# dluvizon/deephar

Hardware: AMD Instinct MI355X
Metric: frames/sec whole-node, 256x256 MPII pose fwd (higher is better)
Workload: dtype f32; 1 GPU; MPII single-person 256x256, ReceptionNet 8 blocks J=16 ctx=2 k=5, pose-only forward, batch=64 per GPU (BASELINE.json configs[1]); global_batch=64, parallelism=frame-shard x1 (replicas, no collective), hipgraph=True, streams=1, input=f32, gemm=f32, outputs_finite_in_range=True

## Files before the change

### deephar_amd/csrc/conv_common.h

```cpp
#pragma once
#include <type_traits>

#include "dh_kernels.h"

namespace dh {

typedef float f32x16 __attribute__((ext_vector_type(16)));
typedef float f32x4v __attribute__((ext_vector_type(4)));

__device__ __forceinline__ void st4_stream(float* ptr, float4 v) {
  f32x4v t = {v.x, v.y, v.z, v.w};
  __builtin_nontemporal_store(t, reinterpret_cast<f32x4v*>(ptr));
}
__device__ __forceinline__ float4 ld4_stream(const float* ptr) {
  const f32x4v t = __builtin_nontemporal_load(reinterpret_cast<const f32x4v*>(ptr));
  return make_float4(t.x, t.y, t.z, t.w);
}

template <typename RSRC>
__device__ __forceinline__ float buf_ld1_stream(RSRC rs, int voff, int soff) {
  float r = 0.f;
#if defined(__HIP_DEVICE_COMPILE__)
  r = __uint_as_float(__builtin_amdgcn_raw_buffer_load_b32(rs, voff, soff, 2));
#endif
  return r;
}
template <typename RSRC>
__device__ __forceinline__ void buf_st1_stream(RSRC rs, int voff, int soff, float v) {
#if defined(__HIP_DEVICE_COMPILE__)
  __builtin_amdgcn_raw_buffer_store_b32(__float_as_uint(v), rs, voff, soff, 2);
#endif
}
__device__ __forceinline__ float& f4c(float4& v, int c) { return c == 0 ? v.x : c == 1 ? v.y : c == 2 ? v.z : v.w; }
__device__ __forceinline__ float f4c(const float4& v, int c) { return c == 0 ? v.x : c == 1 ? v.y : c == 2 ? v.z : v.w; }

__device__ __forceinline__ int xcd_tile(int b, int nwg) {
  const int xcd = b & 7, q = nwg >> 3, r = nwg & 7;
  return (xcd < r ? xcd * (q + 1) : r * (q + 1) + (xcd - r) * q) + (b >> 3);
}

template <int TM, int TN>
struct EpiPrefetch {
  static constexpr int ROW4 = TN * 8;
  static constexpr int IT = 4 * TN;
  static constexpr bool kEnabled = (TM == 1);
  float4 r1[kEnabled ? TM : 1][kEnabled ? IT : 1];
  float dsc[kEnabled ? TN : 1], dsh[kEnabled ? TN : 1];

  template <int WM, int WN>
  static __device__ __forceinline__ bool direct_tile(const ConvArgs& p, int m0, int n0, int M, int epi_vec) {
    return (epi_vec & 2) != 0 && m0 + WM * TM * 32 <= M && n0 + WN * TN * 32 <= p.Cout;
  }

  template <int WM, int WN>
  __device__ __forceinline__ void issue(const ConvArgs& p, int m0, int n0, int M, int epi_vec) {
    if constexpr (kEnabled) {
      if (direct_tile<WM, WN>(p, m0, n0, M, epi_vec)) {
        const int lane = threadIdx.x & 63, wave = threadIdx.x >> 6;
        const int wm = wave / WN, wn = wave % WN;
        const int li = lane & 31, lh = lane >> 5;
        const int ncol = n0 + wn * TN * 32 + li;
        if (p.post_scale != nullptr) {
#pragma unroll
          for (int j = 0; j < TN; ++j) { dsc[j] = p.post_scale[ncol + j * 32]; dsh[j] = p.post_shift[ncol + j * 32]; }
        }
        if (p.res1 == nullptr) return;
        const auto rs = __builtin_amdgcn_make_buffer_rsrc(const_cast<float*>(p.res1), 0,
                                                          (int)(((unsigned)(M - 1) * p.ldr1 + (unsigned)p.Cout) * 4u), 0x00020000);
        const int vo = ((m0 + wm * TM * 32 + 4 * lh) * p.ldr1 + ncol) * 4;
#pragma unroll
        for (int i = 0; i < TM; ++i)
#pragma unroll
          for (int j = 0; j < TN; ++j)
#pragma unroll
            for (int r = 0; r < 16; ++r)
              f4c(r1[i][j * 4 + (r >> 2)], r & 3) = buf_ld1_stream(rs, vo, ((i * 32 + (r & 3) + 8 * (r >> 2)) * p.ldr1 + j * 32) * 4);
        return;
      }
      if (epi_vec == 0 || p.res1 == nullptr) return;
      const int lane = threadIdx.x & 63, wave = threadIdx.x >> 6;
      const int wm = wave / WN, wn = wave % WN;
#pragma unroll
      for (int i = 0; i < TM; ++i)
#pragma unroll
        for (int it = 0; it < IT; ++it) {
          const int f = lane + 64 * it;
          const int row = f / ROW4, c4 = f - row * ROW4;
          int m = m0 + (wm * TM + i) * 32 + row;
          int n = n0 + wn * TN * 32 + c4 * 4;
          m = m < M ? m : M - 1;
          n = n < p.Cout ? n : p.Cout - 4;
          r1[i][it] = ld4_stream(p.res1 + (size_t)m * p.ldr1 + n);
        }
    }
  }
};

struct EpiNoHook {
  __device__ __forceinline__ void operator()() const {}
};

template <int WM, int WN, int TM, int TN, bool UP2, bool PRE, typename HOOK = EpiNoHook, bool DIRECT_R2 = true, int CHROWS = 0>
__device__ __forceinline__ void conv_epilogue(const ConvArgs& p, f32x16 (&acc)[TM][TN], float* smem, int m0,
                                              int n0, int M, int epi_vec, const EpiPrefetch<TM, TN>& pre,
                                              HOOK staged = HOOK()) {
  const int tid = threadIdx.x;
  const int lane = tid & 63;
  const int wave = tid >> 6;
  const int wm = wave / WN, wn = wave % WN;
  const int li = lane & 31, lh = lane >> 5;
  constexpr int LDC = TN * 32 + 4;
  constexpr int ROW4 = TN * 8;
  constexpr int IT = 4 * TN;
  constexpr int NSC = (64 % ROW4 == 0) ? 1 : 3;
  constexpr bool kPre = PRE && EpiPrefetch<TM, TN>::kEnabled;
  constexpr bool kPool = tile_pools_in_pairs(WM, TM, UP2);
  constexpr bool kPoolWave = tile_pools_in_wave(TM, UP2);
  if constexpr (!UP2 && kPre && std::is_same<HOOK, EpiNoHook>::value) {
    if (EpiPrefetch<TM, TN>::template direct_tile<WM, WN>(p, m0, n0, M, epi_vec)) {
      const auto rs_y = __builtin_amdgcn_make_buffer_rsrc(p.y, 0, (int)(((unsigned)(M - 1) * p.ldy + (unsigned)p.Cout) * 4u),
                                                          0x00020000);
      const int ncol = n0 + wn * TN * 32 + li;
      const int vo = ((m0 + wm * TM * 32 + 4 * lh) * p.ldy + ncol) * 4;
      float sc[TN], sh[TN];
#pragma unroll
      for (int j = 0; j < TN; ++j) {
        sc[j] = pre.dsc[j];
        sh[j] = pre.dsh[j];
      }
      float r2[DIRECT_R2 ? TN : 1][8];
      if (DIRECT_R2 && p.res2 != nullptr) {
        const auto rs_2 = __builtin_amdgcn_make_buffer_rsrc(
            const_cast<float*>(p.res2), 0, (int)(((unsigned)((M >> 2) - 1) * p.ldr2 + (unsigned)p.Cout) * 4u), 0x00020000);
        const int ohw = p.OH * p.OW, ow_sh = __ffs(p.OW) - 1;
        const int mb = __builtin_amdgcn_readfirstlane(m0 + wm * 32);
        const int fr = mb >> (__ffs(ohw) - 1), pos = mb & (ohw - 1);
        const int oh0 = pos >> ow_sh, ow0 = pos & (p.OW - 1);
        const int v2 = (2 * lh * p.ldr2 + ncol) * 4;
#pragma unroll
        for (int j = 0; j < TN; ++j)
#pragma unroll
          for (int h = 0; h < 8; ++h) {
            const int tr = 2 * (h & 1) + 8 * (h >> 1);
            const int oh = oh0 + (tr >> ow_sh), ow = ow0 + (tr & (p.OW - 1));
            const int src = (fr * (p.OH >> 1) + (oh >> 1)) * (p.OW >> 1) + (ow >> 1);
            r2[j][h] = buf_ld1_stream(rs_2, v2, (src * p.ldr2 + j * 32) * 4);
          }
      }
#pragma unroll
      for (int i = 0; i < TM; ++i)
#pragma unroll
        for (int j = 0; j < TN; ++j)
#pragma unroll
          for (int r = 0; r < 16; ++r) {
            float t = acc[i][j][r];
            if (p.post_scale != nullptr) t = t * sc[j] + sh[j];
            if (p.res1 != nullptr) t += f4c(pre.r1[i][j * 4 + (r >> 2)], r & 3);
            if (DIRECT_R2 && p.res2 != nullptr) t += r2[DIRECT_R2 ? j : 0][r >> 1];
            if (p.post_relu) t = fmaxf(t, 0.f);
            buf_st1_stream(rs_y, vo, ((i * 32 + (r & 3) + 8 * (r >> 2)) * p.ldy + j * 32) * 4, t);
          }
      return;
    }
  }
  float* sC = smem + wave * 32 * LDC;
  const int ohw = p.OH * p.OW;
  const bool vec = epi_vec != 0;
  const bool pow2 = (p.OW & (p.OW - 1)) == 0 && (ohw & (ohw - 1)) == 0;
  const int ow_sh = __ffs(p.OW) - 1, ohw_sh = __ffs(ohw) - 1;
  __syncthreads();
#pragma unroll
  for (int i = 0; i < TM; ++i) {
    if (i > 0) asm volatile("s_waitcnt lgkmcnt(0)" ::: "memory");
#pragma unroll
    for (int j = 0; j < TN; ++j)
#pragma unroll
      for (int r = 0; r < 16; ++r)
        sC[((r & 3) + 8 * (r >> 2) + 4 * lh) * LDC + j * 32 + li] = acc[i][j][r];
    asm volatile("s_waitcnt lgkmcnt(0)" ::: "memory");
    if (i == TM - 1) staged();
    if (vec) {
      float4 rr[kPre ? 1 : IT], sc[NSC], sh[NSC];
      int ncol[NSC];
#pragma unroll
      for (int q = 0; q < NSC; ++q) {
        const int c4 = (lane + 64 * q) % ROW4;
        const int n = n0 + wn * TN * 32 + c4 * 4;
        ncol[q] = n < p.Cout ? n : p.Cout - 4;
        if (p.post_scale != nullptr) {
          sc[q] = *reinterpret_cast<const float4*>(p.post_scale + ncol[q]);
          sh[q] = *reinterpret_cast<const float4*>(p.post_shift + ncol[q]);
        }
      }
      if constexpr (!kPre && CHROWS == 0) {
        if (p.res1 != nullptr) {
#pragma unroll
          for (int it = 0; it < IT; ++it) {
            const int row = (lane + 64 * it) / ROW4;
            const int m = m0 + (wm * TM + i) * 32 + row;
            rr[it] = ld4_stream(p.res1 + (size_t)(m < M ? m : M - 1) * p.ldr1 + ncol[it % NSC]);
          }
        }
      }
      constexpr int CH = UP2 ? (IT < 4 ? IT : 4) : (CHROWS > 0 && CHROWS < IT ? CHROWS : IT);
      static_assert(IT % CH == 0, "chunks of equal size");
      constexpr int ND = UP2 ? 4 : 1;
#pragma unroll
      for (int c0 = 0; c0 < IT; c0 += CH) {
        float4 r2[CH][ND];
        size_t mo[CH][ND];
        if constexpr (!kPre && CHROWS > 0) {
          if (p.res1 != nullptr) {
#pragma unroll
            for (int u = 0; u < CH; ++u) {
              const int row = (lane + 64 * (c0 + u)) / ROW4;
              const int m = m0 + (wm * TM + i) * 32 + row;
              rr[c0 + u] = ld4_stream(p.res1 + (size_t)(m < M ? m : M - 1) * p.ldr1 + ncol[(c0 + u) % NSC]);
            }
          }
        }
#pragma unroll
        for (int u = 0; u < CH; ++u) {
          const int it = c0 + u;
          const int row = (lane + 64 * it) / ROW4;
          const int m = m0 + (wm * TM + i) * 32 + row;
          const int mc = m < M ? m : M - 1;
          if constexpr (UP2) {
            int fr, oh, ow;
            if (pow2) {
              fr = mc >> ohw_sh;
              const int rem = mc & (ohw - 1);
              oh = rem >> ow_sh;
              ow = rem & (p.OW - 1);
            } else {
              fr = mc / ohw;
              const int rem = mc - fr * ohw;
              oh = rem / p.OW;
              ow = rem - oh * p.OW;
            }
#pragma unroll
            for (int d = 0; d < 4; ++d)
              mo[u][d] = ((size_t)fr * 2 * p.OH + 2 * oh + (d >> 1)) * (2 * p.OW) + 2 * ow + (d & 1);
          } else {
            mo[u][0] = (size_t)mc;
          }
          if (p.res2 != nullptr) {
            if (!UP2 && p.res2_down) {
              int fr, oh, ow;
              if (pow2) {
                fr = mc >> ohw_sh;
                const int rem = mc & (ohw - 1);
                oh = rem >> ow_sh;
                ow = rem & (p.OW - 1);
              } else {
                fr = mc / ohw;
                const int rem = mc - fr * ohw;
                oh = rem / p.OW;
                ow = rem - oh * p.OW;
              }
              const size_t mr = ((size_t)fr * (p.OH >> 1) + (oh >> 1)) * (p.OW >> 1) + (ow >> 1);
              r2[u][0] = *reinterpret_cast<const float4*>(p.res2 + mr * p.ldr2 + ncol[it % NSC]);
            } else {
#pragma unroll
              for (int d = 0; d < ND; ++d)
                r2[u][d] = ld4_stream(p.res2 + mo[u][d] * p.ldr2 + ncol[it % NSC]);
            }
          }
        }
#pragma unroll
        for (int u = 0; u < CH; ++u) {
          const int it = c0 + u;
          const int f = lane + 64 * it;
          const int row = f / ROW4, c4 = f - row * ROW4;
          const int m = m0 + (wm * TM + i) * 32 + row;
          const int nc = ncol[it % NSC];
          const bool ok = m < M && n0 + wn * TN * 32 + c4 * 4 < p.Cout;
          float4 t = *reinterpret_cast<const float4*>(&sC[row * LDC + c4 * 4]);
          if (p.post_scale != nullptr) {
            const float4 a = sc[it % NSC], b = sh[it % NSC];
            t.x = t.x * a.x + b.x; t.y = t.y * a.y + b.y; t.z = t.z * a.z + b.z; t.w = t.w * a.w + b.w;
          }
          if (p.res1 != nullptr) {
            float4 r;
            if constexpr (kPre) r = pre.r1[i][it]; else r = rr[it];
            t.x += r.x; t.y += r.y; t.z += r.z; t.w += r.w;
          }
#pragma unroll
          for (int d = 0; d < ND; ++d) {
            float4 o = t;
            if (p.res2 != nullptr) { o.x += r2[u][d].x; o.y += r2[u][d].y; o.z += r2[u][d].z; o.w += r2[u][d].w; }
            if (p.post_relu) {
              o.x = fmaxf(o.x, 0.f); o.y = fmaxf(o.y, 0.f); o.z = fmaxf(o.z, 0.f); o.w = fmaxf(o.w, 0.f);
            }
            if (ok) st4_stream(p.y + mo[u][d] * p.ldy + nc, o);
            if constexpr (kPool || kPoolWave) {
              if (p.y_pool != nullptr) *reinterpret_cast<float4*>(&sC[row * LDC + c4 * 4]) = o;
            }
          }
        }
      }
    } else {
      for (int f = lane; f < 32 * ROW4; f += 64) {
        const int row = f / ROW4, c4 = f - row * ROW4;
        const int m = m0 + (wm * TM + i) * 32 + row;
        const int n = n0 + wn * TN * 32 + c4 * 4;
        if (m >= M || n >= p.Cout) continue;
        const float4 v = *reinterpret_cast<const float4*>(&sC[row * LDC + c4 * 4]);
        size_t mo[4];
        int nout = 1;
        if constexpr (UP2) {
          const int fr = m / ohw;
          const int rem = m - fr * ohw;
          const int oh = rem / p.OW, ow = rem - oh * p.OW;
#pragma unroll
          for (int d = 0; d < 4; ++d)
            mo[d] = ((size_t)fr * 2 * p.OH + 2 * oh + (d >> 1)) * (2 * p.OW) + 2 * ow + (d & 1);
          nout = 4;
        } else {
          mo[0] = (size_t)m;
        }
#pragma unroll
        for (int e = 0; e < 4; ++e) {
          if (n + e >= p.Cout) break;
          float t = (&v.x)[e];
          if (p.post_scale != nullptr) t = t * p.post_scale[n + e] + p.post_shift[n + e];
          if (p.res1 != nullptr) t += p.res1[(size_t)m * p.ldr1 + n + e];
          for (int d = 0; d < nout; ++d) {
            float o = t;
            if (p.res2 != nullptr) {
              size_t mr = mo[d];
              if (!UP2 && p.res2_down) {
                const int fr = m / ohw;
                const int rem = m - fr * ohw;
                const int oh = rem / p.OW, ow = rem - oh * p.OW;
                mr = ((size_t)fr * (p.OH >> 1) + (oh >> 1)) * (p.OW >> 1) + (ow >> 1);
              }
              o += p.res2[mr * p.ldr2 + n + e];
            }
            if (p.post_relu) o = fmaxf(o, 0.f);
            p.y[mo[d] * p.ldy + n + e] = o;
          }
        }
      }
    }
  }
  if constexpr (kPool) {
    if (p.y_pool != nullptr && vec && p.OW == 32) {
      __syncthreads();
      const float* sE = smem + ((wm & ~1) * WN + wn) * 32 * LDC;
      const float* sO = sE + WN * 32 * LDC;
      const int r_img = m0 / 32 + (wm & ~1);
      if ((r_img + 2) * 32 <= M) {
        const int fr = r_img / p.OH, oh = r_img - fr * p.OH;
        const size_t pp = ((size_t)fr * (p.OH / 2) + oh / 2) * 16;
        for (int idx = (wm & 1) * 64 + lane; idx < 16 * ROW4; idx += 128) {
          const int q = idx / ROW4, c4 = idx - q * ROW4;
          const int n = n0 + wn * TN * 32 + c4 * 4;
          if (n >= p.Cout) continue;
          const float4 a = *reinterpret_cast<const float4*>(&sE[(2 * q) * LDC + c4 * 4]);
          const float4 b = *reinterpret_cast<const float4*>(&sE[(2 * q + 1) * LDC + c4 * 4]);
          const float4 c = *reinterpret_cast<const float4*>(&sO[(2 * q) * LDC + c4 * 4]);
          const float4 d = *reinterpret_cast<const float4*>(&sO[(2 * q + 1) * LDC + c4 * 4]);
          float4 t;
          t.x = fmaxf(fmaxf(a.x, b.x), fmaxf(c.x, d.x)); t.y = fmaxf(fmaxf(a.y, b.y), fmaxf(c.y, d.y));
          t.z = fmaxf(fmaxf(a.z, b.z), fmaxf(c.z, d.z)); t.w = fmaxf(fmaxf(a.w, b.w), fmaxf(c.w, d.w));
          *reinterpret_cast<float4*>(p.y_pool + (pp + q) * p.ldyp + n) = t;
        }
      }
      __syncthreads();
    }
  }
  if constexpr (kPoolWave) {
    if (p.y_pool != nullptr && vec && p.OW < 32) {
      asm volatile("s_waitcnt lgkmcnt(0)" ::: "memory");
      const int mb = m0 + wm * 32;
      if (mb + 32 <= M) {
        const int pw_sh = __ffs(p.OW) - 2;
        const int row0 = mb >> (pw_sh + 1);
        const int fr = row0 / p.OH, oh = row0 - fr * p.OH;
        const size_t pp = ((size_t)fr * (p.OH >> 1) + (oh >> 1)) << pw_sh;
        for (int idx = lane; idx < 8 * ROW4; idx += 64) {
          const int q = idx / ROW4, c4 = idx - q * ROW4;
          const int n = n0 + wn * TN * 32 + c4 * 4;
          if (n >= p.Cout) continue;
          const int pr = q >> pw_sh, pc = q & ((1 << pw_sh) - 1);
          const float* s0 = sC + ((2 * pr) * p.OW + 2 * pc) * LDC + c4 * 4;
          const float4 a = *reinterpret_cast<const float4*>(s0);
          const float4 b = *reinterpret_cast<const float4*>(s0 + LDC);
          const float4 c = *reinterpret_cast<const float4*>(s0 + p.OW * LDC);
          const float4 d = *reinterpret_cast<const float4*>(s0 + (p.OW + 1) * LDC);
          float4 t;
          t.x = fmaxf(fmaxf(a.x, b.x), fmaxf(c.x, d.x)); t.y = fmaxf(fmaxf(a.y, b.y), fmaxf(c.y, d.y));
          t.z = fmaxf(fmaxf(a.z, b.z), fmaxf(c.z, d.z)); t.w = fmaxf(fmaxf(a.w, b.w), fmaxf(c.w, d.w));
          *reinterpret_cast<float4*>(p.y_pool + (pp + q) * p.ldyp + n) = t;
        }
      }
      asm volatile("s_waitcnt lgkmcnt(0)" ::: "memory");
    }
  }
}

template <int WM, int WN, int TM, int TN>
__device__ __forceinline__ void d2s_epilogue(const ConvArgs& p, f32x16 (&acc)[TM][TN], float* smem, const int m0, const int n0,
                                             const int M, const int vec, const int cb) {
  const int lane = threadIdx.x & 63, wave = threadIdx.x >> 6;
  const int wm = wave / WN, wn = wave % WN;
  const int li = lane & 31, lh = lane >> 5;
  constexpr int LDC = TN * 32 + 4, ROW4 = TN * 8, IT = 4 * TN;
  float* sC = smem + wave * 32 * LDC;
  const int hw = p.OH * p.OW;
  const bool pow2 = (p.OW & (p.OW - 1)) == 0 && (hw & (hw - 1)) == 0;
  const int ow_sh = __ffs(p.OW) - 1, hw_sh = __ffs(hw) - 1;
  auto out_pixel = [&](int m, int q) {
    int fr, oh, ow;
    if (pow2) {
      fr = m >> hw_sh;
      const int rem = m & (hw - 1);
      oh = rem >> ow_sh;
      ow = rem & (p.OW - 1);
    } else {
      fr = m / hw;
      const int rem = m - fr * hw;
      oh = rem / p.OW;
      ow = rem - oh * p.OW;
    }
    return ((size_t)fr * 2 * p.OH + 2 * oh + (q >> 1)) * (2 * p.OW) + 2 * ow + (q & 1);
  };
  __syncthreads();
#pragma unroll
  for (int i = 0; i < TM; ++i) {
    if (i > 0) asm volatile("s_waitcnt lgkmcnt(0)" ::: "memory");
#pragma unroll
    for (int j = 0; j < TN; ++j)
#pragma unroll
      for (int r = 0; r < 16; ++r) sC[((r & 3) + 8 * (r >> 2) + 4 * lh) * LDC + j * 32 + li] = acc[i][j][r];
    asm volatile("s_waitcnt lgkmcnt(0)" ::: "memory");
    if (vec) {
      constexpr int CH = IT < 4 ? IT : 4;
#pragma unroll
      for (int c0 = 0; c0 < IT; c0 += CH) {
        float4 rr[CH];
        size_t mo[CH];
        int co[CH];
        bool ok[CH];
#pragma unroll
        for (int u = 0; u < CH; ++u) {
          const int f = lane + 64 * (c0 + u);
          const int row = f / ROW4, c4 = f - row * ROW4;
          const int m = m0 + (wm * TM + i) * 32 + row;
          const int n = n0 + wn * TN * 32 + c4 * 4;
          ok[u] = m < M && n < p.Cout;
          const int mc = ok[u] ? m : 0, nc = ok[u] ? n : 0;
          const int q = (nc >= cb) + (nc >= 2 * cb) + (nc >= 3 * cb);
          co[u] = nc - q * cb;
          mo[u] = out_pixel(mc, q);
          if (p.res1 != nullptr) rr[u] = ld4_stream(p.res1 + mo[u] * p.ldr1 + co[u]);
        }
#pragma unroll
        for (int u = 0; u < CH; ++u) {
          const int f = lane + 64 * (c0 + u);
          const int row = f / ROW4, c4 = f - row * ROW4;
          float4 t = *reinterpret_cast<const float4*>(&sC[row * LDC + c4 * 4]);
          if (p.res1 != nullptr) { t.x += rr[u].x; t.y += rr[u].y; t.z += rr[u].z; t.w += rr[u].w; }
          if (p.post_relu) { t.x = fmaxf(t.x, 0.f); t.y = fmaxf(t.y, 0.f); t.z = fmaxf(t.z, 0.f); t.w = fmaxf(t.w, 0.f); }
          if (ok[u]) st4_stream(p.y + mo[u] * p.ldy + co[u], t);
        }
      }
    } else {
      for (int f = lane; f < 32 * TN * 32; f += 64) {
        const int row = f / (TN * 32), c = f - row * (TN * 32);
        const int m = m0 + (wm * TM + i) * 32 + row;
        const int n = n0 + wn * TN * 32 + c;
        if (m >= M || n >= p.Cout) continue;
        const int q = (n >= cb) + (n >= 2 * cb) + (n >= 3 * cb);
        const int ch = n - q * cb;
        const size_t mo = out_pixel(m, q);
        float t = sC[row * LDC + c];
        if (p.res1 != nullptr) t += p.res1[mo * p.ldr1 + ch];
        if (p.post_relu) t = fmaxf(t, 0.f);
        p.y[mo * p.ldy + ch] = t;
      }
    }
  }
}

}
```

### deephar_amd/csrc/gemm1x1_body.h

```cpp
#pragma once
#include "conv_common.h"
#include "gemm_family.h"
#include "lds_dma.h"

namespace dh {

template <bool PRE, int S>
__device__ __forceinline__ void fetch_affine(unsigned t_sc, unsigned t_sh, float4& sc, float4& sh) {
  if constexpr (PRE) {
    sc = lds_rd<S * 32>(t_sc);
    sh = lds_rd<S * 32>(t_sh);
  }
}

template <int TM, int TN, int BN, int BOFF, int S>
__device__ __forceinline__ void fetch_frags(const unsigned (&a_addr)[TM][4], unsigned b_addr, float4 (&fa)[TM],
                                            float4 (&fb)[TN]) {
  fa[0] = lds_rd<0>(a_addr[0][S]);
  if constexpr (TM > 1) fa[1] = lds_rd<0>(a_addr[1][S]);
  constexpr int BO = BOFF + S * 2 * BN * 16;
  fb[0] = lds_rd<BO>(b_addr);
  if constexpr (TN > 1) fb[1] = lds_rd<BO + 512>(b_addr);
  if constexpr (TN > 2) fb[2] = lds_rd<BO + 1024>(b_addr);
}

template <int WM, int WN, int TM, int TN, bool UP2, bool RELU, bool KXK = false, bool PRE = false, bool D2S = false>
__device__ __forceinline__ void gemm1x1_body(const ConvArgs& p, const int epi_vec, const int block, const int nblocks,
                                             float* const smem, const int cb = 0) {
  static_assert(!(PRE && (KXK || UP2)), "the BN prologue is built for the plain pointwise form");
  static_assert(!(D2S && (KXK || UP2)), "the depth-to-space epilogue follows the plain pointwise main loop");
  constexpr int NT = WM * WN * 64;
  constexpr int BM = WM * TM * 32;
  constexpr int BN = WN * TN * 32;
  constexpr int APASS = BM * 8 / NT;
  constexpr int BPASS = 8 * BN / NT;
  constexpr int STAGE = BM * BK + BK * BN;
  static_assert(BM * 8 % NT == 0 && (8 * BN) % NT == 0, "tile/thread mismatch");

  const int tid = threadIdx.x;
  const int lane = tid & 63;
  const int wave = tid >> 6;
  const int wm = wave / WN, wn = wave % WN;
  const int li = lane & 31, lh = lane >> 5;

  const int M = p.N * p.OH * p.OW;
  const int tiles_n = (p.Cout + BN - 1) / BN;
  const int tile = xcd_tile(block, nblocks);
  const int m0 = (tile / tiles_n) * BM;
  const int n0 = (tile % tiles_n) * BN;

  const int wave_u = __builtin_amdgcn_readfirstlane(wave);
  const auto rs_x = __builtin_amdgcn_make_buffer_rsrc(
      const_cast<float*>(p.x), 0, (int)(((unsigned)(p.N * p.H * p.W - 1) * p.ldx + (unsigned)p.Cin) * 4u), 0x00020000);
  const auto rs_w = __builtin_amdgcn_make_buffer_rsrc(const_cast<float*>(p.w), 0, (int)((unsigned)p.Kp * p.Np * 4u),
                                                      0x00020000);
  unsigned a_off[APASS];
  int a_slot[APASS];
  int a_pix[KXK ? APASS : 1], a_ih0[KXK ? APASS : 1], a_iw0[KXK ? APASS : 1];
#pragma unroll
  for (int ps = 0; ps < APASS; ++ps) {
    const int r = (tid >> 3) + ps * (NT / 8);
    int m = m0 + r;
    m = m < M ? m : M - 1;
    a_slot[ps] = ((tid & 7) ^ (r & 7)) * 4;
    if constexpr (KXK) {
      const int n = m / (p.OH * p.OW);
      const int rem = m - n * (p.OH * p.OW);
      const int oh = rem / p.OW, ow = rem - oh * p.OW;
      a_pix[ps] = n * p.H * p.W;
      a_ih0[ps] = oh * p.SH - p.PT;
      a_iw0[ps] = ow * p.SW - p.PL;
      a_off[ps] = 0;
    } else {
      a_off[ps] = ((unsigned)m * p.ldx + a_slot[ps]) * 4u;
    }
  }
  const int chunks_per_tap = KXK ? p.Cin / BK : 1;
  unsigned b_off[BPASS];
#pragma unroll
  for (int q = 0; q < BPASS; ++q) {
    const int idx = tid + q * NT;
    const int kq = idx / BN, j = idx - kq * BN;
    const int col = n0 + j < p.Np ? n0 + j : 0;
    b_off[q] = ((unsigned)kq * p.Np + col) * 16u;
  }
  const int b_step = 8 * p.Np * 16;

  auto issue = [&](int kt, int stage) {
    float* sA = smem + stage * STAGE;
    float* sB = sA + BM * BK;
    int kh = 0, kw = 0, c0 = 0;
    if constexpr (KXK) {
      const int tap = kt / chunks_per_tap;
      c0 = (kt - tap * chunks_per_tap) * BK;
      kh = tap / p.KW;
      kw = tap - kh * p.KW;
    }
#pragma unroll
    for (int ps = 0; ps < APASS; ++ps) {
      if constexpr (KXK) {
        const int ih = a_ih0[ps] + kh, iw = a_iw0[ps] + kw;
        const bool ok = (unsigned)ih < (unsigned)p.H && (unsigned)iw < (unsigned)p.W && kt * BK < p.K;
        const unsigned off = ok ? ((unsigned)(a_pix[ps] + ih * p.W + iw) * p.ldx + c0 + a_slot[ps]) * 4u : OOB;
        dma16(rs_x, sA + (ps * NT + wave_u * 64) * 4, off, 0);
      } else {
        dma16(rs_x, sA + (ps * NT + wave_u * 64) * 4, a_off[ps], kt * BK * 4);
      }
    }
#pragma unroll
    for (int q = 0; q < BPASS; ++q) dma16(rs_w, sB + (q * NT + wave_u * 64) * 4, b_off[q], kt * b_step);
  };

  f32x16 acc[TM][TN];
#pragma unroll
  for (int i = 0; i < TM; ++i)
#pragma unroll
    for (int j = 0; j < TN; ++j)
#pragma unroll
      for (int r = 0; r < 16; ++r) acc[i][j][r] = 0.f;

  const int nk = p.Kp / BK;
  issue(0, 0);
  if constexpr (PRE) {
    float* tab = smem + 2 * STAGE;
    for (int i = tid; i < p.Kp; i += NT) {
      tab[i] = i < p.K ? p.pre_scale[i] : 0.f;
      tab[p.Kp + i] = i < p.K ? p.pre_shift[i] : 0.f;
    }
  }
  asm volatile("s_waitcnt vmcnt(0)" ::: "memory");
  __syncthreads();

  const unsigned lds0 = (unsigned)(uintptr_t)(lptr_t)smem;
  unsigned a_base[TM][4];
#pragma unroll
  for (int i = 0; i < TM; ++i)
#pragma unroll
    for (int q = 0; q < 4; ++q)
      a_base[i][q] = lds0 + (unsigned)(((wm * TM + i) * 32 + li) * BK * 4 + (((q * 2 + lh) ^ (li & 7)) << 4));
  const unsigned b_base = lds0 + (unsigned)((lh * BN + wn * TN * 32 + li) * 16);
  constexpr int BOFF = BM * BK * 4;

  auto mfma_block = [&](const float4 (&a)[TM], const float4 (&b)[TN]) {
#pragma unroll
    for (int i = 0; i < TM; ++i)
#pragma unroll
      for (int j = 0; j < TN; ++j) {
        acc[i][j] = __builtin_amdgcn_mfma_f32_32x32x2f32(a[i].x, b[j].x, acc[i][j], 0, 0, 0);
        acc[i][j] = __builtin_amdgcn_mfma_f32_32x32x2f32(a[i].y, b[j].y, acc[i][j], 0, 0, 0);
        acc[i][j] = __builtin_amdgcn_mfma_f32_32x32x2f32(a[i].z, b[j].z, acc[i][j], 0, 0, 0);
        acc[i][j] = __builtin_amdgcn_mfma_f32_32x32x2f32(a[i].w, b[j].w, acc[i][j], 0, 0, 0);
      }
  };
  auto relu_frags = [&](float4 (&a)[TM], const float4& sc, const float4& sh) {
    if constexpr (PRE) {
#pragma unroll
      for (int i = 0; i < TM; ++i)
        a[i] = make_float4(fmaf(a[i].x, sc.x, sh.x), fmaf(a[i].y, sc.y, sh.y), fmaf(a[i].z, sc.z, sh.z), fmaf(a[i].w, sc.w, sh.w));
    }
    if constexpr (RELU) {
#pragma unroll
      for (int i = 0; i < TM; ++i) a[i] = relu4(a[i]);
    }
  };
  const unsigned t_sc0 = lds0 + (unsigned)(2 * STAGE * 4 + lh * 16);

  EpiPrefetch<TM, TN> pre;
  for (int kt = 0; kt < nk; ++kt) {
    const int cur = kt & 1;
    if constexpr (!D2S) {
      if (kt == nk - 1) pre.template issue<WM, WN>(p, m0, n0, M, epi_vec);
    }
    const unsigned so = (unsigned)(cur * STAGE * 4);
    unsigned a_addr[TM][4];
#pragma unroll
    for (int i = 0; i < TM; ++i)
#pragma unroll
      for (int q = 0; q < 4; ++q) a_addr[i][q] = a_base[i][q] + so;
    const unsigned b_addr = b_base + so;

    float4 fa0[TM], fb0[TN], fa1[TM], fb1[TN];
    float4 sc0, sh0, sc1, sh1;
    const unsigned t_sc = t_sc0 + (unsigned)(kt * BK * 4), t_sh = t_sc + (unsigned)(p.Kp * 4);
    fetch_frags<TM, TN, BN, BOFF, 0>(a_addr, b_addr, fa0, fb0);
    fetch_affine<PRE, 0>(t_sc, t_sh, sc0, sh0);
    __builtin_amdgcn_sched_barrier(0);
    if (kt + 1 < nk) issue(kt + 1, cur ^ 1);
    lgkm_wait();
    fetch_frags<TM, TN, BN, BOFF, 1>(a_addr, b_addr, fa1, fb1);
    fetch_affine<PRE, 1>(t_sc, t_sh, sc1, sh1);
    __builtin_amdgcn_sched_barrier(0);
    relu_frags(fa0, sc0, sh0);
    mfma_block(fa0, fb0);
    lgkm_wait();
    fetch_frags<TM, TN, BN, BOFF, 2>(a_addr, b_addr, fa0, fb0);
    fetch_affine<PRE, 2>(t_sc, t_sh, sc0, sh0);
    __builtin_amdgcn_sched_barrier(0);
    relu_frags(fa1, sc1, sh1);
    mfma_block(fa1, fb1);
    lgkm_wait();
    fetch_frags<TM, TN, BN, BOFF, 3>(a_addr, b_addr, fa1, fb1);
    fetch_affine<PRE, 3>(t_sc, t_sh, sc1, sh1);
    __builtin_amdgcn_sched_barrier(0);
    relu_frags(fa0, sc0, sh0);
    mfma_block(fa0, fb0);
    lgkm_wait();
    relu_frags(fa1, sc1, sh1);
    mfma_block(fa1, fb1);

    asm volatile("s_waitcnt vmcnt(0)" ::: "memory");
    __syncthreads();
  }

  if constexpr (D2S) d2s_epilogue<WM, WN, TM, TN>(p, acc, smem, m0, n0, M, epi_vec, cb);
  else conv_epilogue<WM, WN, TM, TN, UP2, true>(p, acc, smem, m0, n0, M, epi_vec, pre);
}

}
```

### deephar_amd/csrc/gemm_family.h

```cpp
#pragma once
#include <algorithm>
#include <utility>

#include "conv_rules.h"

namespace dh {

struct GemmLds { size_t launch, limit; };

constexpr int gemm_epi_floats(int WM, int WN, int TN) { return WM * WN * 32 * (TN * 32 + 4); }
constexpr GemmLds gemm_lds(int stage, int epi, bool PRE, int Kp, bool limit_adds_tables) {
  const size_t lds = (size_t)(stage > epi ? stage : epi) * sizeof(float);
  const size_t launch = PRE ? std::max(lds, (size_t)(stage + 2 * Kp) * sizeof(float)) : lds;
  const size_t limit = !PRE ? lds
                       : limit_adds_tables ? lds + 2 * kMaxPreKp * sizeof(float)
                                           : std::max(lds, (size_t)(stage + 2 * kMaxPreKp) * sizeof(float));
  return {launch, limit};
}
constexpr GemmLds gemm_f32_lds(int WM, int WN, int TM, int TN, bool PRE, int Kp) {
  return gemm_lds(2 * (WM * TM * 32 * BK + BK * WN * TN * 32), gemm_epi_floats(WM, WN, TN), PRE, Kp, true);
}
constexpr GemmLds gemm_split_lds(int P, int WM, int WN, int TM, int TN, int NS, bool PRE, int Kp) {
  return gemm_lds(NS * (WM * TM * 32 * BK + 4 * P * WN * TN * 32 * 4), gemm_epi_floats(WM, WN, TN), PRE, Kp, false);
}
constexpr size_t kMaxLds = 160 * 1024;

struct GemmTile {
  int wm, wn, tm, tn, ns;
  bool wide;
  constexpr int bm() const { return wm * tm * 32; }
  constexpr int bn() const { return wn * tn * 32; }
};
constexpr GemmTile kGemmTiles[] = {
    {2, 2, 2, 3, 2},
    {2, 2, 2, 2, 2},
    {4, 1, 1, 3, 2},
    {4, 1, 1, 2, 2},
    {4, 1, 1, 1, 2},
    {2, 1, 1, 3, 2},
    {2, 1, 1, 2, 2},
    {2, 1, 1, 1, 2},
    {1, 1, 1, 1, 2},
    {8, 1, 1, 3, 3},
    {4, 1, 1, 3, 3},
    {8, 1, 1, 2, 3},
    {4, 2, 1, 3, 2},
    {4, 2, 2, 3, 2},
    {4, 1, 1, 6, 2, true},
    {2, 1, 1, 6, 2, true},
};
constexpr int kNumF32Cfgs = 9;
constexpr int kNumSplitCfgs = sizeof(kGemmTiles) / sizeof(kGemmTiles[0]);
constexpr int kNumConvCfgs = 2 * kNumF32Cfgs;

constexpr bool tile_pools_in_pairs(int WM, int TM, bool UP2 = false) { return TM == 1 && WM % 2 == 0 && !UP2; }
constexpr bool tile_pools_in_wave(int TM, bool UP2 = false) { return TM == 1 && !UP2; }
constexpr bool tile_pools_for(const GemmTile& t, int OW) { return OW == 32 ? tile_pools_in_pairs(t.wm, t.tm) : tile_pools_in_wave(t.tm); }
constexpr bool tile_has_up2(const GemmTile& t) { return t.wide || t.tm * t.tn < 6; }
constexpr bool tile_has_parts(const GemmTile& t, int P, bool ext) { return !t.wide || (P == 3 && !ext); }
constexpr bool tile_has_ext_prologue(const GemmTile& t) { return t.tm == 1; }
constexpr bool tile_ext_fits(const GemmTile& t, int P, bool PRE) {
  return gemm_split_lds(P, t.wm, t.wn, t.tm, t.tn, t.ns, PRE, 0).limit <= kMaxLds;
}

template <int... I, typename F>
int dispatch_tile_seq(int cfg, std::integer_sequence<int, I...>, F&& f) {
  int rc = DH_EINVAL;
  (void)((cfg == I && (rc = f(std::integral_constant<int, I>{}), true)) || ...);
  return rc;
}
template <int N, typename F>
int dispatch_tile(int cfg, F&& f) {
  return dispatch_tile_seq(cfg, std::make_integer_sequence<int, N>{}, static_cast<F&&>(f));
}

}
```

Before: 5116 frames/s.

## Peel last K-tile and interleave per-column-slice epilogue with final MFMAs

For TM==1 gemm tiles on direct-store paths, the last K iteration is peeled out of the main loop. The epilogue loads (BN scale/shift, residual 1 and 2) for the next column slice are issued while that slice's final MFMAs run, and each finished slice is stored right away. The aim is to hide epilogue global-load latency behind tensor compute and to lower register pressure from prefetching all residuals at once. The cost is more template complexity and extra code paths whose selection depends on tile and PRE/KXK flags.

```diff
diff --git a/deephar_amd/csrc/conv_common.h b/deephar_amd/csrc/conv_common.h
--- a/deephar_amd/csrc/conv_common.h
+++ b/deephar_amd/csrc/conv_common.h
@@ -52,10 +52,10 @@
     return (epi_vec & 2) != 0 && m0 + WM * TM * 32 <= M && n0 + WN * TN * 32 <= p.Cout;
   }
 
-  template <int WM, int WN>
+  template <int WM, int WN, bool DIRECT = true>
   __device__ __forceinline__ void issue(const ConvArgs& p, int m0, int n0, int M, int epi_vec) {
     if constexpr (kEnabled) {
-      if (direct_tile<WM, WN>(p, m0, n0, M, epi_vec)) {
+      if (DIRECT && direct_tile<WM, WN>(p, m0, n0, M, epi_vec)) {
         const int lane = threadIdx.x & 63, wave = threadIdx.x >> 6;
         const int wm = wave / WN, wn = wave % WN;
         const int li = lane & 31, lh = lane >> 5;
@@ -96,11 +96,105 @@
   }
 };
 
+struct EpiSlice {
+  float r1[16];
+  float r2[8];
+  float sc, sh;
+};
+
+using rsrc_t = decltype(__builtin_amdgcn_make_buffer_rsrc((float*)nullptr, (short)0, 0, 0));
+
+template <int WM, int WN, int TN, bool R2 = true>
+struct EpiDirect {
+  rsrc_t rs_y, rs_1, rs_2;
+  int vo_y, vo_1, vo_2, ncol;
+  int fr, oh0, ow0, ow_sh;
+
+  __device__ __forceinline__ EpiDirect(const ConvArgs& p, int m0, int n0, int M) {
+    const int lane = threadIdx.x & 63, wave = threadIdx.x >> 6;
+    const int wm = wave / WN, wn = wave % WN;
+    const int li = lane & 31, lh = lane >> 5;
+    rs_y = __builtin_amdgcn_make_buffer_rsrc(p.y, 0, (int)(((unsigned)(M - 1) * p.ldy + (unsigned)p.Cout) * 4u), 0x00020000);
+    rs_1 = __builtin_amdgcn_make_buffer_rsrc(const_cast<float*>(p.res1), 0,
+                                             (int)(((unsigned)(M - 1) * p.ldr1 + (unsigned)p.Cout) * 4u), 0x00020000);
+    rs_2 = __builtin_amdgcn_make_buffer_rsrc(const_cast<float*>(p.res2), 0,
+                                             (int)(((unsigned)((M >> 2) - 1) * p.ldr2 + (unsigned)p.Cout) * 4u), 0x00020000);
+    ncol = n0 + wn * TN * 32 + li;
+    const int row0 = m0 + wm * 32 + 4 * lh;
+    vo_y = (row0 * p.ldy + ncol) * 4;
+    vo_1 = (row0 * p.ldr1 + ncol) * 4;
+    vo_2 = (2 * lh * p.ldr2 + ncol) * 4;
+    const int ohw = p.OH * p.OW;
+    const int mb = __builtin_amdgcn_readfirstlane(m0 + wm * 32);
+    const int pos = mb & (ohw - 1);
+    ow_sh = __ffs(p.OW) - 1;
+    fr = mb >> (__ffs(ohw) - 1);
+    oh0 = pos >> ow_sh;
+    ow0 = pos & (p.OW - 1);
+  }
+
+  __device__ __forceinline__ void request_bn(const ConvArgs& p, int j, EpiSlice& s) const {
+    if (p.post_scale != nullptr) {
+      s.sc = p.post_scale[ncol + j * 32];
+      s.sh = p.post_shift[ncol + j * 32];
+    }
+  }
+  __device__ __forceinline__ void request_res1(const ConvArgs& p, int j, EpiSlice& s) const {
+    if (p.res1 != nullptr) {
+#pragma unroll
+      for (int r = 0; r < 16; ++r) s.r1[r] = buf_ld1_stream(rs_1, vo_1, (((r & 3) + 8 * (r >> 2)) * p.ldr1 + j * 32) * 4);
+    }
+  }
+  __device__ __forceinline__ void request_res2(const ConvArgs& p, int j, EpiSlice& s) const {
+    if (R2 && p.res2 != nullptr) {
+#pragma unroll
+      for (int h = 0; h < 8; ++h) {
+        const int tr = 2 * (h & 1) + 8 * (h >> 1);
+        const int oh = oh0 + (tr >> ow_sh), ow = ow0 + (tr & (p.OW - 1));
+        const int src = (fr * (p.OH >> 1) + (oh >> 1)) * (p.OW >> 1) + (ow >> 1);
+        s.r2[h] = buf_ld1_stream(rs_2, vo_2, (src * p.ldr2 + j * 32) * 4);
+      }
+    }
+  }
+  __device__ __forceinline__ void request(const ConvArgs& p, int j, EpiSlice& s) const {
+    request_bn(p, j, s);
+    request_res1(p, j, s);
+    request_res2(p, j, s);
+  }
+
+  __device__ __forceinline__ void finish(const ConvArgs& p, int j, const f32x16& acc, const EpiSlice& s) const {
+    float t[16];
+#pragma unroll
+    for (int r = 0; r < 16; ++r) t[r] = acc[r];
+    if (p.post_scale != nullptr) {
+#pragma unroll
+      for (int r = 0; r < 16; ++r) t[r] = t[r] * s.sc + s.sh;
+    }
+    if (p.res1 != nullptr) {
+#pragma unroll
+      for (int r = 0; r < 16; ++r) t[r] += s.r1[r];
+    }
+    if (R2 && p.res2 != nullptr) {
+#pragma unroll
+      for (int r = 0; r < 16; ++r) t[r] += s.r2[r >> 1];
+    }
+    if (p.post_relu) {
+#pragma unroll
+      for (int r = 0; r < 16; ++r) t[r] = fmaxf(t[r], 0.f);
+    }
+#pragma unroll
+    for (int r = 0; r < 16; ++r) buf_st1_stream(rs_y, vo_y, (((r & 3) + 8 * (r >> 2)) * p.ldy + j * 32) * 4, t[r]);
+  }
+};
+
+enum { kDirectNone = 0, kDirectWhole = 1, kDirectSlices = 2 };
+
 struct EpiNoHook {
   __device__ __forceinline__ void operator()() const {}
 };
 
-template <int WM, int WN, int TM, int TN, bool UP2, bool PRE, typename HOOK = EpiNoHook, bool DIRECT_R2 = true, int CHROWS = 0>
+template <int WM, int WN, int TM, int TN, bool UP2, bool PRE, typename HOOK = EpiNoHook, bool DIRECT_R2 = true, int CHROWS = 0,
+          int DIRECT = kDirectWhole>
 __device__ __forceinline__ void conv_epilogue(const ConvArgs& p, f32x16 (&acc)[TM][TN], float* smem, int m0,
                                               int n0, int M, int epi_vec, const EpiPrefetch<TM, TN>& pre,
                                               HOOK staged = HOOK()) {
@@ -116,50 +210,65 @@
   constexpr bool kPre = PRE && EpiPrefetch<TM, TN>::kEnabled;
   constexpr bool kPool = tile_pools_in_pairs(WM, TM, UP2);
   constexpr bool kPoolWave = tile_pools_in_wave(TM, UP2);
-  if constexpr (!UP2 && kPre && std::is_same<HOOK, EpiNoHook>::value) {
+  if constexpr (DIRECT != kDirectNone && !UP2 && kPre && std::is_same<HOOK, EpiNoHook>::value) {
     if (EpiPrefetch<TM, TN>::template direct_tile<WM, WN>(p, m0, n0, M, epi_vec)) {
-      const auto rs_y = __builtin_amdgcn_make_buffer_rsrc(p.y, 0, (int)(((unsigned)(M - 1) * p.ldy + (unsigned)p.Cout) * 4u),
-                                                          0x00020000);
-      const int ncol = n0 + wn * TN * 32 + li;
-      const int vo = ((m0 + wm * TM * 32 + 4 * lh) * p.ldy + ncol) * 4;
-      float sc[TN], sh[TN];
-#pragma unroll
-      for (int j = 0; j < TN; ++j) {
-        sc[j] = pre.dsc[j];
-        sh[j] = pre.dsh[j];
-      }
-      float r2[DIRECT_R2 ? TN : 1][8];
-      if (DIRECT_R2 && p.res2 != nullptr) {
-        const auto rs_2 = __builtin_amdgcn_make_buffer_rsrc(
-            const_cast<float*>(p.res2), 0, (int)(((unsigned)((M >> 2) - 1) * p.ldr2 + (unsigned)p.Cout) * 4u), 0x00020000);
-        const int ohw = p.OH * p.OW, ow_sh = __ffs(p.OW) - 1;
-        const int mb = __builtin_amdgcn_readfirstlane(m0 + wm * 32);
-        const int fr = mb >> (__ffs(ohw) - 1), pos = mb & (ohw - 1);
-        const int oh0 = pos >> ow_sh, ow0 = pos & (p.OW - 1);
-        const int v2 = (2 * lh * p.ldr2 + ncol) * 4;
-#pragma unroll
-        for (int j = 0; j < TN; ++j)
-#pragma unroll
-          for (int h = 0; h < 8; ++h) {
-            const int tr = 2 * (h & 1) + 8 * (h >> 1);
-            const int oh = oh0 + (tr >> ow_sh), ow = ow0 + (tr & (p.OW - 1));
-            const int src = (fr * (p.OH >> 1) + (oh >> 1)) * (p.OW >> 1) + (ow >> 1);
-            r2[j][h] = buf_ld1_stream(rs_2, v2, (src * p.ldr2 + j * 32) * 4);
-          }
-      }
-#pragma unroll
-      for (int i = 0; i < TM; ++i)
-#pragma unroll
-        for (int j = 0; j < TN; ++j)
-#pragma unroll
-          for (int r = 0; r < 16; ++r) {
-            float t = acc[i][j][r];
-            if (p.post_scale != nullptr) t = t * sc[j] + sh[j];
-            if (p.res1 != nullptr) t += f4c(pre.r1[i][j * 4 + (r >> 2)], r & 3);
-            if (DIRECT_R2 && p.res2 != nullptr) t += r2[DIRECT_R2 ? j : 0][r >> 1];
-            if (p.post_relu) t = fmaxf(t, 0.f);
-            buf_st1_stream(rs_y, vo, ((i * 32 + (r & 3) + 8 * (r >> 2)) * p.ldy + j * 32) * 4, t);
-          }
+      if constexpr (DIRECT == kDirectSlices) {
+        const EpiDirect<WM, WN, TN, DIRECT_R2> epi(p, m0, n0, M);
+        EpiSlice sl[TN];
+#pragma unroll
+        for (int j = 0; j < TN; ++j) {
+          sl[j].sc = pre.dsc[j];
+          sl[j].sh = pre.dsh[j];
+#pragma unroll
+          for (int r = 0; r < 16; ++r) sl[j].r1[r] = f4c(pre.r1[0][j * 4 + (r >> 2)], r & 3);
+          epi.request_res2(p, j, sl[j]);
+        }
+#pragma unroll
+        for (int j = 0; j < TN; ++j) epi.finish(p, j, acc[0][j], sl[j]);
+      } else {
+        const auto rs_y = __builtin_amdgcn_make_buffer_rsrc(p.y, 0, (int)(((unsigned)(M - 1) * p.ldy + (unsigned)p.Cout) * 4u),
+                                                            0x00020000);
+        const int ncol = n0 + wn * TN * 32 + li;
+        const int vo = ((m0 + wm * TM * 32 + 4 * lh) * p.ldy + ncol) * 4;
+        float sc[TN], sh[TN];
+#pragma unroll
+        for (int j = 0; j < TN; ++j) {
+          sc[j] = pre.dsc[j];
+          sh[j] = pre.dsh[j];
+        }
+        float r2[DIRECT_R2 ? TN : 1][8];
+        if (DIRECT_R2 && p.res2 != nullptr) {
+          const auto rs_2 = __builtin_amdgcn_make_buffer_rsrc(
+              const_cast<float*>(p.res2), 0, (int)(((unsigned)((M >> 2) - 1) * p.ldr2 + (unsigned)p.Cout) * 4u), 0x00020000);
+          const int ohw = p.OH * p.OW, ow_sh = __ffs(p.OW) - 1;
+          const int mb = __builtin_amdgcn_readfirstlane(m0 + wm * 32);
+          const int fr = mb >> (__ffs(ohw) - 1), pos = mb & (ohw - 1);
+          const int oh0 = pos >> ow_sh, ow0 = pos & (p.OW - 1);
+          const int v2 = (2 * lh * p.ldr2 + ncol) * 4;
+#pragma unroll
+          for (int j = 0; j < TN; ++j)
+#pragma unroll
+            for (int h = 0; h < 8; ++h) {
+              const int tr = 2 * (h & 1) + 8 * (h >> 1);
+              const int oh = oh0 + (tr >> ow_sh), ow = ow0 + (tr & (p.OW - 1));
+              const int src = (fr * (p.OH >> 1) + (oh >> 1)) * (p.OW >> 1) + (ow >> 1);
+              r2[j][h] = buf_ld1_stream(rs_2, v2, (src * p.ldr2 + j * 32) * 4);
+            }
+        }
+#pragma unroll
+        for (int i = 0; i < TM; ++i)
+#pragma unroll
+          for (int j = 0; j < TN; ++j)
+#pragma unroll
+            for (int r = 0; r < 16; ++r) {
+              float t = acc[i][j][r];
+              if (p.post_scale != nullptr) t = t * sc[j] + sh[j];
+              if (p.res1 != nullptr) t += f4c(pre.r1[i][j * 4 + (r >> 2)], r & 3);
+              if (DIRECT_R2 && p.res2 != nullptr) t += r2[DIRECT_R2 ? j : 0][r >> 1];
+              if (p.post_relu) t = fmaxf(t, 0.f);
+              buf_st1_stream(rs_y, vo, ((i * 32 + (r & 3) + 8 * (r >> 2)) * p.ldy + j * 32) * 4, t);
+            }
+      }
       return;
     }
   }
diff --git a/deephar_amd/csrc/gemm1x1_body.h b/deephar_amd/csrc/gemm1x1_body.h
--- a/deephar_amd/csrc/gemm1x1_body.h
+++ b/deephar_amd/csrc/gemm1x1_body.h
@@ -22,6 +22,21 @@
   fb[0] = lds_rd<BO>(b_addr);
   if constexpr (TN > 1) fb[1] = lds_rd<BO + 512>(b_addr);
   if constexpr (TN > 2) fb[2] = lds_rd<BO + 1024>(b_addr);
+}
+
+template <int I0, int N, typename F>
+__device__ __forceinline__ void static_for(F&& f) {
+  if constexpr (I0 < N) {
+    f(std::integral_constant<int, I0>{});
+    static_for<I0 + 1, N>(f);
+  }
+}
+
+template <int N>
+__device__ __forceinline__ void lgkm_wait_n() {
+  __builtin_amdgcn_sched_barrier(0);
+  asm volatile("s_waitcnt lgkmcnt(%0)" ::"n"(N) : "memory");
+  __builtin_amdgcn_sched_barrier(0);
 }
 
 template <int WM, int WN, int TM, int TN, bool UP2, bool RELU, bool KXK = false, bool PRE = false, bool D2S = false>
@@ -166,10 +181,13 @@
   const unsigned t_sc0 = lds0 + (unsigned)(2 * STAGE * 4 + lh * 16);
 
   EpiPrefetch<TM, TN> pre;
-  for (int kt = 0; kt < nk; ++kt) {
+  constexpr bool kSliced = tile_epi_sliced(GemmTile{WM, WN, TM, TN}, PRE, KXK) && !UP2 && !D2S;
+  const bool sliced = kSliced && EpiPrefetch<TM, TN>::template direct_tile<WM, WN>(p, m0, n0, M, epi_vec);
+  const int nloop = sliced ? nk - 1 : nk;
+  for (int kt = 0; kt < nloop; ++kt) {
     const int cur = kt & 1;
     if constexpr (!D2S) {
-      if (kt == nk - 1) pre.template issue<WM, WN>(p, m0, n0, M, epi_vec);
+      if (kt == nk - 1) pre.template issue<WM, WN, !kSliced>(p, m0, n0, M, epi_vec);
     }
     const unsigned so = (unsigned)(cur * STAGE * 4);
     unsigned a_addr[TM][4];
@@ -212,8 +230,68 @@
     __syncthreads();
   }
 
+  if constexpr (kSliced) {
+    if (sliced) {
+      const int kt = nk - 1;
+      const unsigned so = (unsigned)((kt & 1) * STAGE * 4);
+      const unsigned b_addr = b_base + so;
+      const unsigned t_sc = t_sc0 + (unsigned)(kt * BK * 4), t_sh = t_sc + (unsigned)(p.Kp * 4);
+      const EpiDirect<WM, WN, TN> epi(p, m0, n0, M);
+      EpiSlice sl[2];
+      epi.request(p, 0, sl[0]);
+      float4 fa[4][1], fb[4], sc[4], sh[4];
+      auto read_a = [&](auto sc_) {
+        constexpr int S = decltype(sc_)::value;
+        fa[S][0] = lds_rd<0>(a_base[0][S] + so);
+        fetch_affine<PRE, S>(t_sc, t_sh, sc[S], sh[S]);
+      };
+      auto read_b0 = [&](auto sc_) {
+        constexpr int S = decltype(sc_)::value;
+        fb[S] = lds_rd<BOFF + S * 2 * BN * 16>(b_addr);
+      };
+      if constexpr (PRE) {
+        read_a(std::integral_constant<int, 0>{});
+        static_for<0, 3>([&](auto sc_) {
+          constexpr int S = decltype(sc_)::value;
+          read_a(std::integral_constant<int, S + 1>{});
+          lgkm_wait_n<3>();
+          relu_frags(fa[S], sc[S], sh[S]);
+        });
+        static_for<0, 4>(read_b0);
+        lgkm_wait_n<4>();
+        relu_frags(fa[3], sc[3], sh[3]);
+        lgkm_wait();
+      } else {
+        static_for<0, 4>(read_a);
+        static_for<0, 4>(read_b0);
+        lgkm_wait();
+        static_for<0, 4>([&](auto sc_) { relu_frags(fa[decltype(sc_)::value], sc[0], sh[0]); });
+      }
+      static_for<0, TN>([&](auto jc) {
+        constexpr int J = decltype(jc)::value;
+        if constexpr (J + 1 < TN) epi.request(p, J + 1, sl[(J + 1) & 1]);
+        __builtin_amdgcn_sched_barrier(0);
+        static_for<0, 4>([&](auto sc_) {
+          constexpr int S = decltype(sc_)::value;
+          acc[0][J] = __builtin_amdgcn_mfma_f32_32x32x2f32(fa[S][0].x, fb[S].x, acc[0][J], 0, 0, 0);
+          acc[0][J] = __builtin_amdgcn_mfma_f32_32x32x2f32(fa[S][0].y, fb[S].y, acc[0][J], 0, 0, 0);
+          acc[0][J] = __builtin_amdgcn_mfma_f32_32x32x2f32(fa[S][0].z, fb[S].z, acc[0][J], 0, 0, 0);
+          acc[0][J] = __builtin_amdgcn_mfma_f32_32x32x2f32(fa[S][0].w, fb[S].w, acc[0][J], 0, 0, 0);
+          if constexpr (J + 1 < TN) {
+            __builtin_amdgcn_sched_barrier(0);
+            fb[S] = lds_rd<BOFF + S * 2 * BN * 16 + (J + 1) * 512>(b_addr);
+            __builtin_amdgcn_sched_barrier(0);
+          }
+        });
+        if constexpr (J + 1 < TN) lgkm_wait();
+        epi.finish(p, J, acc[0][J], sl[J & 1]);
+      });
+      return;
+    }
+  }
+  constexpr int kDirect = kSliced ? kDirectNone : kDirectSlices;
   if constexpr (D2S) d2s_epilogue<WM, WN, TM, TN>(p, acc, smem, m0, n0, M, epi_vec, cb);
-  else conv_epilogue<WM, WN, TM, TN, UP2, true>(p, acc, smem, m0, n0, M, epi_vec, pre);
-}
-
-}
+  else conv_epilogue<WM, WN, TM, TN, UP2, true, EpiNoHook, true, 0, kDirect>(p, acc, smem, m0, n0, M, epi_vec, pre);
+}
+
+}
diff --git a/deephar_amd/csrc/gemm_family.h b/deephar_amd/csrc/gemm_family.h
--- a/deephar_amd/csrc/gemm_family.h
+++ b/deephar_amd/csrc/gemm_family.h
@@ -56,6 +56,9 @@
 constexpr bool tile_pools_in_pairs(int WM, int TM, bool UP2 = false) { return TM == 1 && WM % 2 == 0 && !UP2; }
 constexpr bool tile_pools_in_wave(int TM, bool UP2 = false) { return TM == 1 && !UP2; }
 constexpr bool tile_pools_for(const GemmTile& t, int OW) { return OW == 32 ? tile_pools_in_pairs(t.wm, t.tm) : tile_pools_in_wave(t.tm); }
+constexpr bool tile_epi_sliced(const GemmTile& t, bool PRE = false, bool KXK = false) {
+  return t.tm == 1 && !(PRE && t.tn < 3) && !(KXK && t.wm == 1 && t.tn == 1);
+}
 constexpr bool tile_has_up2(const GemmTile& t) { return t.wide || t.tm * t.tn < 6; }
 constexpr bool tile_has_parts(const GemmTile& t, int P, bool ext) { return !t.wide || (P == 3 && !ext); }
 constexpr bool tile_has_ext_prologue(const GemmTile& t) { return t.tm == 1; }
```

New measurement: 5194 frames/s (median of 6 runs). 1.5% higher.
